# iamgroot42/A-LINK

Measured on AMD Instinct MI355X. Metric: 112x112 face embeddings/sec (IR-ResNet-100 ArcFace, 512-d, L2-normalised), higher is better.
Workload: dtype bf16

## Files before the change

a-link_amd/csrc/conv_igemm.hip:

```cpp
#include "conv_device.h"

namespace alink {

namespace {

template <typename T, int WP, int WC, bool DMA, bool SP>
__global__ __launch_bounds__(256, 2) void conv_igemm_kernel(const ConvParams p) {
    typedef typename Vec8<T>::type vec8;
    constexpr int BM = WP * 64, BN = WC * 64;
    constexpr int PJ = BM / 32, WJ = BN / 32;
    constexpr int TILE_BYTES = (BM + BN) * 128;
    extern __shared__ __attribute__((aligned(16))) char smem[];

    const int tid  = threadIdx.x;
    const int lane = tid & 63;
    const int wave = __builtin_amdgcn_readfirstlane(tid >> 6);
    const int wp = wave / WC, wc = wave % WC;

    const int ntn = p.Cout / BN;
    const int nwg = gridDim.x;
    const int lid = xcd_remap(blockIdx.x, nwg);
    const int tile_n = lid % ntn, tile_m = lid / ntn;
    const int m0 = tile_m * BM, n0 = tile_n * BN;
    const int split = blockIdx.y;

    const int Cin = p.Cin, W = p.W, ksz = p.ksz;
    const int CinP = SP ? 2 * Cin : Cin;
    const int Cin2 = SP ? 0 : p.Cin2;
    const int K = (SP ? 2 : 1) * ksz * ksz * Cin + Cin2;
    const int cpt = Cin >> 6;
    const int cpt2 = Cin2 >> 6;
    const int ntap = ksz * ksz;
    const int nk = ntap * cpt * (SP ? 3 : 1) + cpt2;
    const int kt0 = split * p.ksteps_per_split;
    const int kt1 = min(kt0 + p.ksteps_per_split, nk);

    const T* __restrict__ gin = (const T*)p.in;
    const T* __restrict__ gin2 = (const T*)p.in2;
    const T* __restrict__ gw  = (const T*)p.wgt;
    const T* __restrict__ gz  = (const T*)p.zero;

    const int chunk = (tid & 7) ^ ((tid >> 4) & 7);
    int      poff[PJ], poff2[PJ];
    unsigned pmask[PJ];
    {
        const int HoWo = p.Ho * p.Wo;
#pragma unroll
        for (int j = 0; j < PJ; ++j) {
            const int m = m0 + (tid >> 3) + 32 * j;
            unsigned mask = 0;
            int off = 0;
            poff2[j] = -1;
            if (m < p.M) {
                const int n = m / HoWo, rem = m - n * HoWo;
                const int oy = rem / p.Wo, ox = rem - oy * p.Wo;
                const int iy0 = oy * p.stride - p.pad, ix0 = ox * p.stride - p.pad;
                off = ((n * p.H + iy0) * W + ix0) * CinP + chunk * 8;
                poff2[j] = (p.in2_compact ? m : (n * p.H + oy * p.stride) * W + ox * p.stride) * Cin2 + chunk * 8;
                for (int ky = 0; ky < ksz; ++ky)
                    for (int kx = 0; kx < ksz; ++kx)
                        if ((unsigned)(iy0 + ky) < (unsigned)p.H && (unsigned)(ix0 + kx) < (unsigned)W)
                            mask |= 1u << (ky * ksz + kx);
            }
            poff[j] = off;
            pmask[j] = mask;
        }
    }
    int woff[WJ];
#pragma unroll
    for (int j = 0; j < WJ; ++j) woff[j] = (n0 + (tid >> 3) + 32 * j) * K + chunk * 8;

    const int r0 = SP ? kt0 / 3 : kt0;
    int s_ph = SP ? kt0 - 3 * r0 : 0;
    int s_tap = r0 / cpt, s_cc = r0 - s_tap * cpt;
    int s_ky = s_tap / ksz, s_kx = s_tap - s_ky * ksz;

    auto stage = [&](int buf, int kt) {
        char* base = smem + buf * TILE_BYTES;
        const int tap_off = (s_ky * W + s_kx) * CinP + (SP ? 2 * s_cc + (s_ph == 2 ? 1 : 0) : s_cc) * 64;
        const int wk_off = SP ? ((s_tap * cpt + s_cc) * 2 + (s_ph == 1 ? 1 : 0)) * 64 : kt * 64;
        const bool shortcut = !SP && s_tap == ntap;
#pragma unroll
        for (int j = 0; j < PJ; ++j) {
            const bool ok = shortcut ? poff2[j] >= 0 : (pmask[j] >> s_tap) & 1u;
            const T* src = ok ? (shortcut ? gin2 + (poff2[j] + s_cc * 64) : gin + (poff[j] + tap_off)) : gz + (tid & 7) * 8;
            if constexpr (DMA) {
                dma16(src, base + (wave * 8 + 32 * j) * 128);
            } else {
                *(uint4*)(base + ((tid >> 3) + 32 * j) * 128 + (tid & 7) * 16) = *(const uint4*)src;
            }
        }
        char* wbase = base + BM * 128;
#pragma unroll
        for (int j = 0; j < WJ; ++j) {
            const T* src = gw + (woff[j] + wk_off);
            if constexpr (DMA) {
                dma16(src, wbase + (wave * 8 + 32 * j) * 128);
            } else {
                *(uint4*)(wbase + ((tid >> 3) + 32 * j) * 128 + (tid & 7) * 16) = *(const uint4*)src;
            }
        }
        if (SP && ++s_ph < 3) return;
        s_ph = 0;
        if (++s_cc == (shortcut ? cpt2 : cpt)) {
            s_cc = 0;
            ++s_tap;
            if (++s_kx == ksz) { s_kx = 0; ++s_ky; }
        }
    };

    const int q = lane >> 4, lr = lane & 15;
    const int sw = lr >> 1;
    const int foff0 = lr * 128 + (((0 | q) ^ sw) << 4);
    const int foff1 = lr * 128 + (((4 | q) ^ sw) << 4);

    f32x4 acc[4][4];
#pragma unroll
    for (int t = 0; t < 4; ++t)
#pragma unroll
        for (int u = 0; u < 4; ++u) acc[t][u] = f32x4{0.f, 0.f, 0.f, 0.f};

    auto mma = [&](const char* pb, const char* wb) {
#pragma unroll
        for (int ks = 0; ks < 2; ++ks) {
            const int fo = ks ? foff1 : foff0;
            vec8 wf[4], pf[4];
#pragma unroll
            for (int t = 0; t < 4; ++t) wf[t] = *(const vec8*)(wb + t * 2048 + fo);
#pragma unroll
            for (int u = 0; u < 4; ++u) pf[u] = *(const vec8*)(pb + u * 2048 + fo);
#pragma unroll
            for (int t = 0; t < 4; ++t)
#pragma unroll
                for (int u = 0; u < 4; ++u) acc[t][u] = mfma16<T>(wf[t], pf[u], acc[t][u]);
        }
    };
    if constexpr (SP) {
        char* const A0 = smem, * const W0 = smem + BM * 128, * const A1 = smem + TILE_BYTES, * const W1 = smem + TILE_BYTES + BM * 128;
        auto stage_a = [&](char* dst, int part) {
            const int tap_off = (s_ky * W + s_kx) * CinP + (2 * s_cc + part) * 64;
#pragma unroll
            for (int j = 0; j < PJ; ++j) {
                const bool ok = (pmask[j] >> s_tap) & 1u;
                dma16(ok ? gin + (poff[j] + tap_off) : gz + (tid & 7) * 8, dst + (wave * 8 + 32 * j) * 128);
            }
        };
        auto stage_w = [&](char* dst, int blk) {
            const int wk_off = ((s_tap * cpt + s_cc) * 2 + blk) * 64;
#pragma unroll
            for (int j = 0; j < WJ; ++j) dma16(gw + (woff[j] + wk_off), dst + (wave * 8 + 32 * j) * 128);
        };
        auto advance = [&]() {
            if (++s_cc == cpt) {
                s_cc = 0;
                ++s_tap;
                if (++s_kx == ksz) { s_kx = 0; ++s_ky; }
            }
        };
        const int r1 = kt1 / 3;
        if (p.nprod == 1) {
            if (r0 < r1) {
                stage_a(A1, 0);
                stage_w(W0, 0);
                __syncthreads();
                for (int r = r0; r < r1; ++r) {
                    const bool odd = (r - r0) & 1;
                    advance();
                    if (r + 1 < r1) {
                        stage_a(odd ? A1 : A0, 0);
                        stage_w(odd ? W0 : W1, 0);
                    }
                    mma((odd ? A0 : A1) + (wp * 64) * 128, (odd ? W1 : W0) + (wc * 64) * 128);
                    __syncthreads();
                }
            }
        } else
        if (r0 < r1) {
            stage_a(A0, 1);
            stage_w(W0, 0);
            __syncthreads();
            const char* const pa0 = A0 + (wp * 64) * 128, * const pa1 = A1 + (wp * 64) * 128;
            const char* const pw0 = W0 + (wc * 64) * 128, * const pw1 = W1 + (wc * 64) * 128;
            for (int r = r0; r < r1; ++r) {
                stage_a(A1, 0);
                mma(pa0, pw0);
                __syncthreads();
                stage_w(W1, 1);
                mma(pa1, pw0);
                __syncthreads();
                advance();
                if (r + 1 < r1) {
                    stage_a(A0, 1);
                    stage_w(W0, 0);
                }
                mma(pa1, pw1);
                __syncthreads();
            }
        }
    } else
    if (kt0 < kt1) {
        stage(0, kt0);
        __syncthreads();
        for (int kt = kt0; kt < kt1; ++kt) {
            const int cur = (kt - kt0) & 1;
            if (kt + 1 < kt1) stage(cur ^ 1, kt + 1);
            mma(smem + cur * TILE_BYTES + (wp * 64) * 128, smem + cur * TILE_BYTES + (BM + wc * 64) * 128);
            __syncthreads();
        }
    }

    const int cbase = n0 + wc * 64 + 16 * q;
    if (p.splitk > 1) {
        float* slab = (float*)p.out + (size_t)split * p.M * p.Cout;
#pragma unroll
        for (int u = 0; u < 4; ++u) {
            const int m = m0 + wp * 64 + 16 * u + lr;
            if (m < p.M) {
                float* o = slab + (size_t)m * p.Cout + cbase;
#pragma unroll
                for (int t = 0; t < 4; ++t) *(f32x4*)(o + 4 * t) = acc[t][u];
            }
        }
        return;
    }

    const int HoWo = p.Ho * p.Wo;
    size_t off[4];
    bool ok[4];
    int cls[4];
#pragma unroll
    for (int u = 0; u < 4; ++u) {
        const int m = m0 + wp * 64 + 16 * u + lr;
        ok[u] = m < p.M;
        const int mc = ok[u] ? m : p.M - 1;
        off[u] = SP ? (size_t)mc * (2 * p.Cout) + (size_t)(cbase >> 6) * 128 + (cbase & 63) : (size_t)mc * p.Cout + cbase;
        cls[u] = 0;
        if (p.border_cls) {
            const int rem = mc % HoWo;
            const int oy = rem / p.Wo, ox = rem - oy * p.Wo;
            const int rc = (oy == 0) ? 0 : ((oy == p.Ho - 1) ? 2 : 1);
            const int cc = (ox == 0) ? 0 : ((ox == p.Wo - 1) ? 2 : 1);
            cls[u] = rc * 3 + cc;
        }
    }
    vec8 res[4][SP ? 4 : 2];
    const T* extra = (const T*)(p.dact ? p.dact : p.resid);
    if (extra) {
#pragma unroll
        for (int u = 0; u < 4; ++u) {
            res[u][0] = *(const vec8*)(extra + off[u]);
            res[u][1] = *(const vec8*)(extra + off[u] + 8);
            if (SP) {
                res[u][2] = *(const vec8*)(extra + off[u] + 64);
                res[u][3] = *(const vec8*)(extra + off[u] + 72);
            }
        }
    }
    f32x4 bia[4][4];
#pragma unroll
    for (int u = 0; u < 4; ++u)
#pragma unroll
        for (int t = 0; t < 4; ++t) bia[u][t] = *(const f32x4*)(p.bias + cls[u] * p.Cout + cbase + 4 * t);
    float al[16];
    if (p.alpha) {
#pragma unroll
        for (int t = 0; t < 4; ++t) {
            const f32x4 a4 = *(const f32x4*)(p.alpha + cbase + 4 * t);
#pragma unroll
            for (int j = 0; j < 4; ++j) al[4 * t + j] = a4[j];
        }
    }
#pragma unroll
    for (int u = 0; u < 4; ++u) {
        float v[16];
#pragma unroll
        for (int t = 0; t < 4; ++t)
#pragma unroll
            for (int j = 0; j < 4; ++j)
                v[4 * t + j] = SP ? fmaf(acc[t][u][j], p.acc_scale, bia[u][t][j] * p.bias_scale) : acc[t][u][j] + bia[u][t][j];
        if (!SP && p.dact) {
#pragma unroll
            for (int i = 0; i < 8; ++i) {
                v[i] *= (float)res[u][0][i] > 0.f ? 1.f : al[i];
                v[8 + i] *= (float)res[u][1][i] > 0.f ? 1.f : al[8 + i];
            }
        } else {
            if (p.alpha) {
#pragma unroll
                for (int i = 0; i < 16; ++i) v[i] = v[i] > 0.f ? v[i] : v[i] * al[i];
            }
            if (p.resid) {
#pragma unroll
                for (int i = 0; i < 8; ++i) {
                    if (SP) {
                        v[i] = fmaf((float)res[u][0][i] + (float)res[u][2][i], p.res_scale, v[i]);
                        v[8 + i] = fmaf((float)res[u][1][i] + (float)res[u][3][i], p.res_scale, v[8 + i]);
                    } else {
                        v[i] += (float)res[u][0][i];
                        v[8 + i] += (float)res[u][1][i];
                    }
                }
            }
        }
        if (p.post_relu) {
#pragma unroll
            for (int i = 0; i < 16; ++i) v[i] = relu_keep_nan(v[i]);
        }
        if (ok[u]) {
            vec8 o0, o1;
#pragma unroll
            for (int i = 0; i < 8; ++i) {
                o0[i] = (T)v[i];
                o1[i] = (T)v[8 + i];
            }
            *(vec8*)((T*)p.out + off[u]) = o0;
            *(vec8*)((T*)p.out + off[u] + 8) = o1;
            if (SP) {
                vec8 l0, l1;
#pragma unroll
                for (int i = 0; i < 8; ++i) {
                    l0[i] = (T)(v[i] - (float)o0[i]);
                    l1[i] = (T)(v[8 + i] - (float)o1[i]);
                }
                *(vec8*)((T*)p.out + off[u] + 64) = l0;
                *(vec8*)((T*)p.out + off[u] + 72) = l1;
            }
        }
    }
}

template <typename T, int WP, int WC, bool DMA, bool SP = false>
hipError_t launch_one(const ConvParams& p, hipStream_t stream) {
    constexpr int BM = WP * 64, BN = WC * 64;
    constexpr size_t lds = 2 * (size_t)(BM + BN) * 128;
    const int ntm = (p.M + BM - 1) / BM, ntn = p.Cout / BN;
    dim3 grid(ntm * ntn, p.splitk, 1), block(256, 1, 1);
    hipLaunchKernelGGL((conv_igemm_kernel<T, WP, WC, DMA, SP>), grid, block, lds, stream, p);
    return hipGetLastError();
}

template <typename T, int WP, int WC, bool DMA, bool SP = false>
hipError_t set_attr_one() {
    constexpr size_t lds = 2 * (size_t)(WP * 64 + WC * 64) * 128;
    return hipFuncSetAttribute((const void*)conv_igemm_kernel<T, WP, WC, DMA, SP>,
                               hipFuncAttributeMaxDynamicSharedMemorySize, (int)lds);
}

bool g_use_dma = true;

}

extern "C" void alink_debug_set_dma(int on) { g_use_dma = on != 0; }

hipError_t conv_set_attributes() {
    hipError_t e;
#define A(T, WP, WC)                                                    \
    if ((e = set_attr_one<T, WP, WC, true>()) != hipSuccess) return e;  \
    if ((e = set_attr_one<T, WP, WC, false>()) != hipSuccess) return e;
    A(__bf16, 4, 1) A(__bf16, 2, 2) A(_Float16, 4, 1) A(_Float16, 2, 2)
#undef A
    if ((e = set_attr_one<_Float16, 4, 1, true, true>()) != hipSuccess) return e;
    if ((e = set_attr_one<_Float16, 2, 2, true, true>()) != hipSuccess) return e;
    return hipSuccess;
}

double conv_flops(const ConvParams& p) {
    return 2.0 * (double)p.M * (double)p.Cout * (double)(p.ksz * p.ksz * p.Cin + (p.in2 ? p.Cin2 : 0));
}

hipError_t launch_conv_igemm(int dtype, const ConvParams& p, hipStream_t stream) {
    if (p.Cin % 64 || p.Cout % 64 || p.M <= 0 || p.splitk < 1) return hipErrorInvalidValue;
    if (p.in2 ? (p.Cin2 <= 0 || p.Cin2 % 64 || p.splitk != 1 || dtype == ALINK_DT_F16X2) : p.Cin2 != 0) return hipErrorInvalidValue;
    if ((long long)p.N * p.H * p.W * p.Cin2 >= (1ll << 31)) return hipErrorInvalidValue;
    if (p.ksz * p.ksz > 32) return hipErrorInvalidValue;
    const int two = dtype == ALINK_DT_F16X2 ? 2 : 1;
    if ((long long)p.N * p.H * p.W * p.Cin * two >= (1ll << 31)) return hipErrorInvalidValue;
    if ((long long)p.Cout * p.ksz * p.ksz * p.Cin * two >= (1ll << 31)) return hipErrorInvalidValue;
    if (conv_gemm_lat_applies(dtype, p)) return launch_conv_gemm_lat(dtype, p, stream);
    const bool wide = (p.Cout % 128) == 0;
    if (dtype == ALINK_DT_F16X2) {
        if (p.dact || (p.splitk > 1 && p.ksteps_per_split % 3)) return hipErrorInvalidValue;
        return wide ? launch_one<_Float16, 2, 2, true, true>(p, stream) : launch_one<_Float16, 4, 1, true, true>(p, stream);
    }
#define L(T)                                                                          \
    (wide ? (g_use_dma ? launch_one<T, 2, 2, true>(p, stream)                         \
                       : launch_one<T, 2, 2, false>(p, stream))                       \
          : (g_use_dma ? launch_one<T, 4, 1, true>(p, stream)                         \
                       : launch_one<T, 4, 1, false>(p, stream)))
    if (dtype == ALINK_DT_BF16) return L(__bf16);
    if (dtype == ALINK_DT_F16) return L(_Float16);
#undef L
    return hipErrorInvalidValue;
}

}
```

include/alink_hip_debug.h:

```cpp
#ifndef ALINK_HIP_DEBUG_H
#define ALINK_HIP_DEBUG_H

#include <stddef.h>

#ifdef __cplusplus
extern "C" {
#endif

void alink_debug_set_linear(int mode);
void alink_debug_set_generic_epilogue(int on);
void alink_debug_set_direct(int on);
void alink_debug_set_pair(int on);
void alink_debug_set_c64(int on);
void alink_debug_set_s2direct(int on);
void alink_debug_set_fuse_stem(int on);
void alink_debug_set_fuse_unit(int mode);
void alink_debug_set_fuse_unit1(int mode);
void alink_debug_set_fuse_shortcut(int on);
void alink_debug_set_dma(int on);
void alink_debug_set_fine_max(int n);
void alink_debug_set_sibling_aware(int on);
void alink_debug_set_latency_form(int max_pixels);
void alink_debug_set_latency_tiles(int form);
void alink_debug_set_stagger(int n);
void alink_debug_set_early_refill(int on);
void alink_debug_set_shard_stagger(int on);

void alink_debug_set_tiny_step(int on);
void alink_debug_set_mini_step(int on);
void alink_debug_set_head_bf16_mfma(int on);

void alink_debug_set_smallres_overlap(int on);
void alink_debug_set_smallres_one_update(int on);

void alink_debug_set_stop_after(int n);
void alink_debug_set_profile_reps(int n);
void alink_debug_set_ablate(int a);
void alink_debug_set_stamps(void* dev_u64);
int alink_debug_lds_oob_probe(float* dev_out516, void* stream);
int alink_debug_linear_contract_ok(void);


struct alink_resnet50;
struct alink_backbone;
int alink_debug_resnet50_grad_cache_info(const struct alink_resnet50* r, int n_images, int index, size_t* byte_offset, int* H,
                                         int* W, int* C, char* name_buf, int name_len);
int alink_debug_backbone_grad_cache_info(const struct alink_backbone* bb, int n_images, int index, size_t* byte_offset, int* H,
                                         int* W, int* C, char* name_buf, int name_len);

struct alink_vgg16;
int alink_debug_vgg16_embed_prefix(struct alink_vgg16* r, const float* dev_in, int n_images, int preprocessed, float* dev_out,
                                   void* ws, size_t ws_bytes, void* stream, int n_ops, size_t* byte_offset, int* H, int* W,
                                   int* C, char* name_buf, int name_len, int* kernel, int* form);

int alink_debug_resnet50_embed_prefix(struct alink_resnet50* r, const float* dev_in, int n_images, int preprocessed, float* dev_out,
                                      void* ws, size_t ws_bytes, void* stream, int n_ops, size_t* byte_offset, int* H, int* W,
                                      int* C, char* name_buf, int name_len, int* kernel, int* form, int* scale_exp);

#ifdef __cplusplus
}
#endif
#endif
```

Baseline: 49850.

## Add ENDS variant of igemm conv with cheaper prologue and LDS-staged epilogue tables

Adds an ENDS template variant of the implicit-GEMM conv kernel that is enabled by default. The prologue issues the first weight DMA before the pixel setup and replaces per-row integer divisions with incremental pixel stepping using reciprocal-based small division. The main loop is split into separate tap and shortcut phases with specialised staging. During the last MMA step, the bias and alpha tables are DMA'd into the free LDS buffer so the epilogue reads them from LDS, and the border classes are precomputed. The goal is to shorten the prologue and epilogue latency of each tile, at the cost of more template instantiations and risk from float-based division rounding.

```diff
diff --git a/a-link_amd/csrc/conv_igemm.hip b/a-link_amd/csrc/conv_igemm.hip
--- a/a-link_amd/csrc/conv_igemm.hip
+++ b/a-link_amd/csrc/conv_igemm.hip
@@ -4,12 +4,37 @@
 
 namespace {
 
-template <typename T, int WP, int WC, bool DMA, bool SP>
+template <bool B> struct BoolTag { static constexpr bool value = B; };
+
+struct Pix { int n, oy, ox; };
+struct PixStep { int a, c, d; };
+
+__device__ __forceinline__ int small_div(int x, int d) { return (int)(((float)x + 0.5f) * __builtin_amdgcn_rcpf((float)d)); }
+
+__device__ __forceinline__ PixStep pix_step(int delta, int HoWo, int Wo) {
+    PixStep s;
+    s.a = small_div(delta, HoWo);
+    const int b = delta - s.a * HoWo;
+    s.c = small_div(b, Wo);
+    s.d = b - s.c * Wo;
+    return s;
+}
+
+__device__ __forceinline__ Pix pix_advance(Pix x, PixStep s, int Ho, int Wo) {
+    x.n += s.a; x.oy += s.c; x.ox += s.d;
+    if (x.ox >= Wo) { x.ox -= Wo; ++x.oy; }
+    if (x.oy >= Ho) { x.oy -= Ho; ++x.n; }
+    return x;
+}
+
+template <typename T, int WP, int WC, bool DMA, bool SP, bool ENDS>
 __global__ __launch_bounds__(256, 2) void conv_igemm_kernel(const ConvParams p) {
+    static_assert(!(SP && ENDS), "the split-precision forms keep the first form of the two ends");
     typedef typename Vec8<T>::type vec8;
     constexpr int BM = WP * 64, BN = WC * 64;
     constexpr int PJ = BM / 32, WJ = BN / 32;
     constexpr int TILE_BYTES = (BM + BN) * 128;
+    constexpr int TBL_ROWS = 10;
     extern __shared__ __attribute__((aligned(16))) char smem[];
 
     const int tid  = threadIdx.x;
@@ -41,9 +66,61 @@
     const T* __restrict__ gz  = (const T*)p.zero;
 
     const int chunk = (tid & 7) ^ ((tid >> 4) & 7);
+    int woff[WJ];
+#pragma unroll
+    for (int j = 0; j < WJ; ++j) woff[j] = (n0 + (tid >> 3) + 32 * j) * K + chunk * 8;
+    auto stage_w = [&](int buf, int wk_off) {
+        char* wbase = smem + buf * TILE_BYTES + BM * 128;
+#pragma unroll
+        for (int j = 0; j < WJ; ++j) {
+            const T* src = gw + (woff[j] + wk_off);
+            if constexpr (DMA) {
+                dma16(src, wbase + (wave * 8 + 32 * j) * 128);
+            } else {
+                *(uint4*)(wbase + ((tid >> 3) + 32 * j) * 128 + (tid & 7) * 16) = *(const uint4*)src;
+            }
+        }
+    };
+    const int q = lane >> 4, lr = lane & 15;
+
     int      poff[PJ], poff2[PJ];
     unsigned pmask[PJ];
-    {
+    unsigned clsp = 0;
+    int tbl_buf = 0;
+    Pix tile = {0, 0, 0};
+    if constexpr (ENDS) {
+        if (kt0 < kt1) stage_w(0, kt0 * 64);
+        __builtin_amdgcn_sched_barrier(0);
+        const int Ho = p.Ho, Wo = p.Wo, HoWo = Ho * Wo;
+        tile.n = m0 / HoWo;
+        const int rem0 = m0 - tile.n * HoWo;
+        tile.oy = rem0 / Wo;
+        tile.ox = rem0 - tile.oy * Wo;
+        const PixStep s32 = pix_step(32, HoWo, Wo);
+        Pix x = pix_advance(tile, pix_step(tid >> 3, HoWo, Wo), Ho, Wo);
+        auto tap_mask = [&](auto wide, int iy0, int ix0) {
+            constexpr int KM = decltype(wide)::value ? 5 : 3;
+            unsigned cv = 0, mask = 0;
+#pragma unroll
+            for (int kx = 0; kx < KM; ++kx) cv |= (unsigned)(kx < ksz && (unsigned)(ix0 + kx) < (unsigned)W) << kx;
+#pragma unroll
+            for (int ky = 0; ky < KM; ++ky) mask |= (ky < ksz && (unsigned)(iy0 + ky) < (unsigned)p.H ? cv : 0u) << (ky * ksz);
+            return mask;
+        };
+#pragma unroll
+        for (int j = 0; j < PJ; ++j) {
+            const int m = m0 + (tid >> 3) + 32 * j;
+            const bool valid = m < p.M;
+            const int iy0 = x.oy * p.stride - p.pad, ix0 = x.ox * p.stride - p.pad;
+            const unsigned mask = ksz <= 3 ? tap_mask(BoolTag<false>(), iy0, ix0) : tap_mask(BoolTag<true>(), iy0, ix0);
+            const unsigned pix = (unsigned)(x.n * p.H + iy0) * W + ix0;
+            const unsigned pix2 = p.in2_compact ? (unsigned)m : (unsigned)(x.n * p.H + x.oy * p.stride) * W + x.ox * p.stride;
+            poff[j] = (int)(pix * CinP + chunk * 8);
+            poff2[j] = (int)(pix2 * Cin2 + chunk * 8);
+            pmask[j] = valid ? (mask | 0x80000000u) : 0u;
+            x = pix_advance(x, s32, Ho, Wo);
+        }
+    } else {
         const int HoWo = p.Ho * p.Wo;
 #pragma unroll
         for (int j = 0; j < PJ; ++j) {
@@ -66,14 +143,14 @@
             pmask[j] = mask;
         }
     }
-    int woff[WJ];
-#pragma unroll
-    for (int j = 0; j < WJ; ++j) woff[j] = (n0 + (tid >> 3) + 32 * j) * K + chunk * 8;
 
     const int r0 = SP ? kt0 / 3 : kt0;
     int s_ph = SP ? kt0 - 3 * r0 : 0;
-    int s_tap = r0 / cpt, s_cc = r0 - s_tap * cpt;
-    int s_ky = s_tap / ksz, s_kx = s_tap - s_ky * ksz;
+    int s_tap = 0, s_cc = 0, s_ky = 0, s_kx = 0;
+    if (!ENDS || r0 != 0) {
+        s_tap = r0 / cpt, s_cc = r0 - s_tap * cpt;
+        s_ky = s_tap / ksz, s_kx = s_tap - s_ky * ksz;
+    }
 
     auto stage = [&](int buf, int kt) {
         char* base = smem + buf * TILE_BYTES;
@@ -109,7 +186,51 @@
         }
     };
 
-    const int q = lane >> 4, lr = lane & 15;
+    const T* const zsrc = gz + (tid & 7) * 8;
+    auto stage_px = [&](auto sc, int buf) {
+        constexpr bool SC = decltype(sc)::value;
+        char* base = smem + buf * TILE_BYTES;
+        const int step_off = SC ? s_cc * 64 : (s_ky * W + s_kx) * CinP + s_cc * 64;
+#pragma unroll
+        for (int j = 0; j < PJ; ++j) {
+            const bool ok = SC ? (pmask[j] >> 31) != 0 : ((pmask[j] >> s_tap) & 1u) != 0;
+            const T* in_src = SC ? gin2 + (poff2[j] + step_off) : gin + (poff[j] + step_off);
+            const T* src = ok ? in_src : zsrc;
+            if constexpr (DMA) {
+                dma16(src, base + (wave * 8 + 32 * j) * 128);
+            } else {
+                *(uint4*)(base + ((tid >> 3) + 32 * j) * 128 + (tid & 7) * 16) = *(const uint4*)src;
+            }
+        }
+        ++s_cc;
+        if (!SC && s_cc == cpt) {
+            s_cc = 0;
+            ++s_tap;
+            if (++s_kx == ksz) { s_kx = 0; ++s_ky; }
+        }
+    };
+    auto stage_table = [&](int buf) {
+        char* tb = smem + buf * TILE_BYTES;
+        constexpr int LPR = BN / 4;
+        constexpr int NDMA = (TBL_ROWS * BN * 4 + 1023) / 1024;
+        const int ncls = p.border_cls ? 9 : 1;
+#pragma unroll
+        for (int i = 0; i * 4 < NDMA; ++i) {
+            const int d = wave + 4 * i;
+            if (d < NDMA) {
+                const int l = d * 64 + lane, row = l / LPR, col = l % LPR;
+                const float* src = (const float*)p.zero + (lane & 7) * 4;
+                if (row < ncls) src = p.bias + (row * p.Cout + n0 + col * 4);
+                if (row == TBL_ROWS - 1 && p.alpha) src = p.alpha + (n0 + col * 4);
+                if constexpr (DMA) {
+                    dma16(src, tb + d * 1024);
+                } else {
+                    *(uint4*)(tb + l * 16) = *(const uint4*)src;
+                }
+            }
+        }
+    };
+
     const int sw = lr >> 1;
     const int foff0 = lr * 128 + (((0 | q) ^ sw) << 4);
     const int foff1 = lr * 128 + (((4 | q) ^ sw) << 4);
@@ -197,6 +318,41 @@
                 __syncthreads();
             }
         }
+    } else if constexpr (ENDS) {
+        if (kt0 < kt1) {
+            const int n_tap = min(kt1, ntap * cpt) - kt0, n_sc = kt1 - kt0 - n_tap;
+            stage_px(BoolTag<false>(), 0);
+            __builtin_amdgcn_sched_barrier(0);
+            if (p.border_cls && p.splitk == 1) {
+                const int Ho = p.Ho, Wo = p.Wo, HoWo = Ho * Wo;
+                const PixStep s16 = pix_step(16, HoWo, Wo);
+                Pix e = pix_advance(tile, pix_step(wp * 64 + lr, HoWo, Wo), Ho, Wo);
+#pragma unroll
+                for (int u = 0; u < 4; ++u) {
+                    const int rc = (e.oy == 0) ? 0 : ((e.oy == Ho - 1) ? 2 : 1);
+                    const int cc = (e.ox == 0) ? 0 : ((e.ox == Wo - 1) ? 2 : 1);
+                    clsp |= (unsigned)(rc * 3 + cc) << (4 * u);
+                    e = pix_advance(e, s16, Ho, Wo);
+                }
+            }
+            asm volatile("" : "+v"(clsp));
+            wait_then_barrier<0>();
+            int cur = 0, wk = kt0 * 64;
+            auto step = [&](auto sc) {
+                wk += 64;
+                stage_w(cur ^ 1, wk);
+                stage_px(sc, cur ^ 1);
+                mma(smem + cur * TILE_BYTES + (wp * 64) * 128, smem + cur * TILE_BYTES + (BM + wc * 64) * 128);
+                wait_then_barrier<0>();
+                cur ^= 1;
+            };
+            for (int i = n_tap - 1; i > 0; --i) step(BoolTag<false>());
+            for (int i = n_sc; i > 0; --i) step(BoolTag<true>());
+            if (p.splitk == 1) stage_table(cur ^ 1);
+            mma(smem + cur * TILE_BYTES + (wp * 64) * 128, smem + cur * TILE_BYTES + (BM + wc * 64) * 128);
+            wait_then_barrier<0>();
+            tbl_buf = cur ^ 1;
+        }
     } else
     if (kt0 < kt1) {
         stage(0, kt0);
@@ -234,8 +390,8 @@
         ok[u] = m < p.M;
         const int mc = ok[u] ? m : p.M - 1;
         off[u] = SP ? (size_t)mc * (2 * p.Cout) + (size_t)(cbase >> 6) * 128 + (cbase & 63) : (size_t)mc * p.Cout + cbase;
-        cls[u] = 0;
-        if (p.border_cls) {
+        cls[u] = ENDS ? (clsp >> (4 * u)) & 15u : 0;
+        if (!ENDS && p.border_cls) {
             const int rem = mc % HoWo;
             const int oy = rem / p.Wo, ox = rem - oy * p.Wo;
             const int rc = (oy == 0) ? 0 : ((oy == p.Ho - 1) ? 2 : 1);
@@ -256,16 +412,18 @@
             }
         }
     }
+    const char* const tbl = smem + tbl_buf * TILE_BYTES + (wc * 64 + 16 * q) * 4;
     f32x4 bia[4][4];
 #pragma unroll
     for (int u = 0; u < 4; ++u)
 #pragma unroll
-        for (int t = 0; t < 4; ++t) bia[u][t] = *(const f32x4*)(p.bias + cls[u] * p.Cout + cbase + 4 * t);
+        for (int t = 0; t < 4; ++t)
+            bia[u][t] = ENDS ? *(const f32x4*)(tbl + cls[u] * (BN * 4) + 16 * t) : *(const f32x4*)(p.bias + cls[u] * p.Cout + cbase + 4 * t);
     float al[16];
     if (p.alpha) {
 #pragma unroll
         for (int t = 0; t < 4; ++t) {
-            const f32x4 a4 = *(const f32x4*)(p.alpha + cbase + 4 * t);
+            const f32x4 a4 = ENDS ? *(const f32x4*)(tbl + (TBL_ROWS - 1) * (BN * 4) + 16 * t) : *(const f32x4*)(p.alpha + cbase + 4 * t);
 #pragma unroll
             for (int j = 0; j < 4; ++j) al[4 * t + j] = a4[j];
         }
@@ -329,34 +487,38 @@
     }
 }
 
-template <typename T, int WP, int WC, bool DMA, bool SP = false>
+template <typename T, int WP, int WC, bool DMA, bool SP = false, bool ENDS = false>
 hipError_t launch_one(const ConvParams& p, hipStream_t stream) {
     constexpr int BM = WP * 64, BN = WC * 64;
     constexpr size_t lds = 2 * (size_t)(BM + BN) * 128;
     const int ntm = (p.M + BM - 1) / BM, ntn = p.Cout / BN;
     dim3 grid(ntm * ntn, p.splitk, 1), block(256, 1, 1);
-    hipLaunchKernelGGL((conv_igemm_kernel<T, WP, WC, DMA, SP>), grid, block, lds, stream, p);
+    hipLaunchKernelGGL((conv_igemm_kernel<T, WP, WC, DMA, SP, ENDS>), grid, block, lds, stream, p);
     return hipGetLastError();
 }
 
-template <typename T, int WP, int WC, bool DMA, bool SP = false>
+template <typename T, int WP, int WC, bool DMA, bool SP = false, bool ENDS = false>
 hipError_t set_attr_one() {
     constexpr size_t lds = 2 * (size_t)(WP * 64 + WC * 64) * 128;
-    return hipFuncSetAttribute((const void*)conv_igemm_kernel<T, WP, WC, DMA, SP>,
+    return hipFuncSetAttribute((const void*)conv_igemm_kernel<T, WP, WC, DMA, SP, ENDS>,
                                hipFuncAttributeMaxDynamicSharedMemorySize, (int)lds);
 }
 
 bool g_use_dma = true;
+bool g_ends = true;
 
 }
 
 extern "C" void alink_debug_set_dma(int on) { g_use_dma = on != 0; }
+extern "C" void alink_debug_set_igemm_ends(int on) { g_ends = on != 0; }
 
 hipError_t conv_set_attributes() {
     hipError_t e;
-#define A(T, WP, WC)                                                    \
-    if ((e = set_attr_one<T, WP, WC, true>()) != hipSuccess) return e;  \
-    if ((e = set_attr_one<T, WP, WC, false>()) != hipSuccess) return e;
+#define A(T, WP, WC)                                                                  \
+    if ((e = set_attr_one<T, WP, WC, true, false, false>()) != hipSuccess) return e;  \
+    if ((e = set_attr_one<T, WP, WC, false, false, false>()) != hipSuccess) return e; \
+    if ((e = set_attr_one<T, WP, WC, true, false, true>()) != hipSuccess) return e;   \
+    if ((e = set_attr_one<T, WP, WC, false, false, true>()) != hipSuccess) return e;
     A(__bf16, 4, 1) A(__bf16, 2, 2) A(_Float16, 4, 1) A(_Float16, 2, 2)
 #undef A
     if ((e = set_attr_one<_Float16, 4, 1, true, true>()) != hipSuccess) return e;
@@ -382,14 +544,16 @@
         if (p.dact || (p.splitk > 1 && p.ksteps_per_split % 3)) return hipErrorInvalidValue;
         return wide ? launch_one<_Float16, 2, 2, true, true>(p, stream) : launch_one<_Float16, 4, 1, true, true>(p, stream);
     }
-#define L(T)                                                                          \
-    (wide ? (g_use_dma ? launch_one<T, 2, 2, true>(p, stream)                         \
-                       : launch_one<T, 2, 2, false>(p, stream))                       \
-          : (g_use_dma ? launch_one<T, 4, 1, true>(p, stream)                         \
-                       : launch_one<T, 4, 1, false>(p, stream)))
+#define L2(T, WP, WC)                                                                  \
+    (g_use_dma ? (g_ends ? launch_one<T, WP, WC, true, false, true>(p, stream)         \
+                         : launch_one<T, WP, WC, true, false, false>(p, stream))       \
+               : (g_ends ? launch_one<T, WP, WC, false, false, true>(p, stream)        \
+                         : launch_one<T, WP, WC, false, false, false>(p, stream)))
+#define L(T) (wide ? L2(T, 2, 2) : L2(T, 4, 1))
     if (dtype == ALINK_DT_BF16) return L(__bf16);
     if (dtype == ALINK_DT_F16) return L(_Float16);
 #undef L
+#undef L2
     return hipErrorInvalidValue;
 }
 
diff --git a/include/alink_hip_debug.h b/include/alink_hip_debug.h
--- a/include/alink_hip_debug.h
+++ b/include/alink_hip_debug.h
@@ -18,6 +18,7 @@
 void alink_debug_set_fuse_unit1(int mode);
 void alink_debug_set_fuse_shortcut(int on);
 void alink_debug_set_dma(int on);
+void alink_debug_set_igemm_ends(int on);
 void alink_debug_set_fine_max(int n);
 void alink_debug_set_sibling_aware(int on);
 void alink_debug_set_latency_form(int max_pixels);
```

New measurement: 50230, median of 6. No clear change (+0.8%).
